# zhuzilin/ring-flash-attention

Hardware: NVIDIA B200
Metric: zigzag_ring_flash_attn_qkvpacked_func fwd_bwd iter/s (higher is better)
Workload: dtype bf16

## Files before the change

### ring_flash_attn_b200/csrc/attn_bwd_sm100.cu

```cuda
#include <math_constants.h>
#include <stdio.h>

#include "attn_common.h"
#include "comm_device.cuh"
#include "sm100_ptx.cuh"

namespace rfa {
namespace bwd {

#ifdef RFA_TRACE
#define RFA_STAMP(cond, iter, slot)                                                              \
  do {                                                                                            \
    if ((cond) && cta == 0 && p.trace != nullptr && (iter) < 64) p.trace[(iter)*16 + (slot)] = clock64(); \
  } while (0)
#else
#define RFA_STAMP(cond, iter, slot) \
  do {                              \
  } while (0)
#endif

constexpr int kTileK = 128;
constexpr int kTileQ = 64;
constexpr int kStages = 3;
constexpr int kThreads = 512;
constexpr int kQHalf = kTileQ * 128;
constexpr int kKVHalf = kTileK * 128;
constexpr int kDSBytes = kTileK * kTileQ * 2;
template <int kD>
struct Geo {
  static constexpr int kKVBytes = kTileK * kD * 2;
  static constexpr int kQBytes = kTileQ * kD * 2;
  static constexpr int kDQBytes = kTileQ * kD * 4;
  static constexpr int kSmemBytes = 2 * kKVBytes + kStages * 2 * kQBytes + kDSBytes + kDQBytes +
                                    kStages * 2 * kTileQ * 4  + 1024  + 1024 ;
};
constexpr uint32_t kTmemCols = 512;
constexpr uint32_t kColS = 0, kColDP = 128, kColDQ = 192, kColDV = 256, kColDK = 384;

struct Barriers {
  uint64_t kv_full;
  uint64_t qdo_full[kStages];
  uint64_t qdo_empty[kStages];
  uint64_t stat_full[kStages];
  uint64_t s_full[2];
  uint64_t p_ready[2];
  uint64_t dp_full;
  uint64_t ds_ready;
  uint64_t dq_full;
  uint64_t dq_free;
  uint64_t dkv_done;
  uint32_t tmem_base;
  uint32_t pad;
};

constexpr int kStatBytes = kStages * 2 * kTileQ * 4;

struct QGeom {
  int q_row0, q_len, diag, lo;
  int t_begin, t_end;
};
__device__ __forceinline__ QGeom q_geom(const BwdQSegment& s) {
  QGeom g;
  g.q_row0 = s.q_row0;
  g.q_len = s.q_len;
  g.diag = s.diag;
  g.lo = s.lo;
  const int first = s.diag >= 0 ? 0 : -s.diag;
  g.t_begin = first / kTileQ;
  g.t_end = (s.q_len + kTileQ - 1) / kTileQ;
  if (g.t_begin > g.t_end) g.t_begin = g.t_end;
  return g;
}

template <typename T, bool kWindow, int kD>
__global__ void __launch_bounds__(kThreads, 1)
attn_bwd_kernel(const __grid_constant__ CUtensorMap tm_q, const __grid_constant__ CUtensorMap tm_do,
                const __grid_constant__ CUtensorMap tm_k, const __grid_constant__ CUtensorMap tm_v,
                const __grid_constant__ CUtensorMap tm_ks, const __grid_constant__ CUtensorMap tm_vs,
                const __grid_constant__ CUtensorMap tm_dq, const __grid_constant__ BwdParams p) {
  if (static_cast<int>(blockIdx.x) < p.push.n_ctas) {
    if (p.push.use_tma) {
      extern __shared__ uint8_t push_smem_raw[];
      push_role_tma(p.push, reinterpret_cast<uint8_t*>((reinterpret_cast<uintptr_t>(push_smem_raw) + 1023) & ~uintptr_t(1023)));
    } else {
      push_role(p.push);
    }
    return;
  }
  static_assert(kD == 64 || kD == 128, "head dim 64 or 128");
  constexpr int kKVBytes = Geo<kD>::kKVBytes, kQBytes = Geo<kD>::kQBytes, kDQBytes = Geo<kD>::kDQBytes;
  constexpr int kSubTiles = kD / 64;
  const int cta = static_cast<int>(blockIdx.x) - p.push.n_ctas;
  extern __shared__ uint8_t smem_raw[];
  uint8_t* smem = reinterpret_cast<uint8_t*>((reinterpret_cast<uintptr_t>(smem_raw) + 1023) & ~uintptr_t(1023));
  uint8_t* smem_k = smem;
  uint8_t* smem_v = smem_k + kKVBytes;
  uint8_t* smem_qdo = smem_v + kKVBytes;
  uint8_t* smem_ds = smem_qdo + kStages * 2 * kQBytes;
  float* smem_dq = reinterpret_cast<float*>(smem_ds + kDSBytes);
  float* smem_stat = reinterpret_cast<float*>(reinterpret_cast<uint8_t*>(smem_dq) + kDQBytes);
  Barriers* bars = reinterpret_cast<Barriers*>(reinterpret_cast<uint8_t*>(smem_stat) + kStatBytes);

  const int warp = threadIdx.x >> 5;
  const int lane = threadIdx.x & 31;
  const int kv_head = p.item_major ? cta % p.hkv : cta / p.n_items;
  const int group = p.hq / p.hkv;
  BwdItem it = p.items[p.item_major ? cta / p.hkv : cta % p.n_items];
  if (p.flags & 4) it.seg_count = 0;

  if (warp == 0 && lane == 0) {
    tma_prefetch_desc(&tm_q);
    tma_prefetch_desc(&tm_do);
    tma_prefetch_desc(&tm_k);
    tma_prefetch_desc(&tm_v);
    tma_prefetch_desc(&tm_dq);
    tma_prefetch_desc(&tm_ks);
    tma_prefetch_desc(&tm_vs);
  }
  if (warp == 1 && lane == 0) {
    mbar_init(&bars->kv_full, 1);
    for (int i = 0; i < kStages; ++i) {
      mbar_init(&bars->qdo_full[i], 1);
      mbar_init(&bars->qdo_empty[i], 1);
      mbar_init(&bars->stat_full[i], 1);
    }
    mbar_init(&bars->s_full[0], 1);
    mbar_init(&bars->s_full[1], 1);
    mbar_init(&bars->p_ready[0], 256);
    mbar_init(&bars->p_ready[1], 256);
    mbar_init(&bars->dp_full, 1);
    mbar_init(&bars->ds_ready, 256);
    mbar_init(&bars->dq_full, 1);
    mbar_init(&bars->dq_free, 128);
    mbar_init(&bars->dkv_done, 1);
    fence_mbar_init();
  }
  if (warp == 2) tmem_alloc<kTmemCols>(&bars->tmem_base);
  tc_fence_before();
  __syncthreads();
  tc_fence_after();
  const uint32_t tmem = bars->tmem_base;

  int tiles_per_head = 0;
  for (int si = 0; si < it.seg_count; ++si) {
    const QGeom g = q_geom(p.qsegs[it.seg_begin + si]);
    tiles_per_head += g.t_end - g.t_begin;
  }
  const int total_tiles = tiles_per_head * group;

  if (warp < 4) {
    reg_dealloc<72>();
    if (warp == 0) {
      if (lane == 0 && total_tiles > 0) {
        const bool staged = it.flag >= 0 && p.ready_flags != nullptr;
        if (staged && !(p.flags & 2)) {
          wait_epoch(p.ready_flags + it.flag, p.ready_epoch, "bwd kv ready", p.sig.my_rank, it.flag);
          fence_proxy_async_all();
        }
        const CUtensorMap* mk = staged ? &tm_ks : &tm_k;
        const CUtensorMap* mv = staged ? &tm_vs : &tm_v;
        mbar_arrive_expect_tx(&bars->kv_full, 2 * kKVBytes);
#pragma unroll
        for (int h = 0; h < kSubTiles; ++h) {
          tma_load_3d(smem_k + h * kKVHalf, mk, &bars->kv_full, 64 * h, kv_head, it.kv_row0);
          tma_load_3d(smem_v + h * kKVHalf, mv, &bars->kv_full, 64 * h, kv_head, it.kv_row0);
        }
        uint32_t slot = 0, phase = 0;
        for (int gq = 0; gq < group; ++gq) {
          const int head = kv_head * group + gq;
          for (int si = 0; si < it.seg_count; ++si) {
            const QGeom g = q_geom(p.qsegs[it.seg_begin + si]);
            for (int ti = g.t_begin; ti < g.t_end; ++ti) {
              const int row = g.q_row0 + ti * kTileQ;
              mbar_wait(&bars->qdo_empty[slot], phase ^ 1);
              uint8_t* dq_ = smem_qdo + slot * 2 * kQBytes;
              uint8_t* ddo = dq_ + kQBytes;
              mbar_arrive_expect_tx(&bars->qdo_full[slot], 2 * kQBytes);
#pragma unroll
              for (int h = 0; h < kSubTiles; ++h) {
                tma_load_3d(dq_ + h * kQHalf, &tm_q, &bars->qdo_full[slot], 64 * h, head, row);
                tma_load_3d(ddo + h * kQHalf, &tm_do, &bars->qdo_full[slot], 64 * h, head, row);
              }
              if (++slot == kStages) {
                slot = 0;
                phase ^= 1;
              }
            }
          }
        }
      }
    } else if (warp == 1) {
      if (total_tiles > 0) {
        const bool leader = elect_one();
        constexpr uint32_t fmt = Pack2<T>::kFmt;
        constexpr uint32_t idesc_st = umma_idesc_f16(fmt, kTileK, kTileQ, 0, 0);
        constexpr uint32_t idesc_dv = umma_idesc_f16(fmt, kTileK, kD, 0, 1);
        constexpr uint32_t idesc_dq = umma_idesc_f16(fmt, 128, kTileQ, 1, 1);
        const uint32_t k_base = smem_u32(smem_k), v_base = smem_u32(smem_v);
        const uint32_t qdo_base = smem_u32(smem_qdo), ds_base = smem_u32(smem_ds);

        constexpr uint32_t hi = umma_desc_hi(1024, kSwizzle128B);
        const uint32_t k_km = umma_desc_lo(k_base, 16);
        const uint32_t v_km = umma_desc_lo(v_base, 16);
        const uint32_t k_mn = umma_desc_lo(k_base, kKVHalf);
        const uint32_t ds_km = umma_desc_lo(ds_base, 16);
        const uint32_t q_km0 = umma_desc_lo(qdo_base, 16);
        const uint32_t q_mn0 = umma_desc_lo(qdo_base, kQHalf);
        constexpr uint32_t stage_step = (2 * kQBytes) >> 4, do_step = kQBytes >> 4;

        auto issue_kq = [&](uint32_t d_col, uint32_t a_lo, uint32_t b_lo) {
#pragma unroll
          for (int k = 0; k < kD / 16; ++k) {
            const uint32_t oa = ((k >> 2) * kKVHalf + (k & 3) * 32) >> 4;
            const uint32_t ob = ((k >> 2) * kQHalf + (k & 3) * 32) >> 4;
            umma_ss2(d_col, a_lo + oa, hi, b_lo + ob, hi, idesc_st, k > 0);
          }
        };

        mbar_wait(&bars->kv_full, 0);
        tc_fence_after();

        uint32_t ph_p[2] = {0, 0};
        uint32_t ph_ds = 0, ph_dqfree = 0;
        int issued_s = 0;
        uint32_t s_slot = 0, s_phase = 0;
        auto issue_s = [&]() {
          mbar_wait(&bars->qdo_full[s_slot], s_phase);
          tc_fence_after();
          if (leader) {
            issue_kq(tmem + kColS + (issued_s & 1) * 64, k_km, q_km0 + s_slot * stage_step);
            umma_commit(&bars->s_full[issued_s & 1]);
          }
          ++issued_s;
          if (++s_slot == kStages) {
            s_slot = 0;
            s_phase ^= 1;
          }
        };
        auto issue_dv = [&](int t, uint32_t t_slot) {
          mbar_wait(&bars->p_ready[t & 1], ph_p[t & 1]);
          ph_p[t & 1] ^= 1;
          tc_fence_after();
          const uint32_t do_mn = q_mn0 + t_slot * stage_step + do_step;
          if (leader)
#pragma unroll
            for (int k = 0; k < kTileQ / 16; ++k)
              umma_ts2(tmem + kColDV, tmem + kColS + (t & 1) * 64 + (k >> 1) * 32 + (k & 1) * 8,
                       do_mn + k * (2048 >> 4), hi, idesc_dv, (t > 0 || k > 0) ? 1u : 0u);
        };
        auto next_slot = [](uint32_t sl) { return sl + 1 == kStages ? 0u : sl + 1; };

        issue_s();
        if (leader) {
          issue_kq(tmem + kColDP, v_km, q_km0 + do_step);
          umma_commit(&bars->dp_full);
        }
        if (total_tiles > 1) issue_s();
        issue_dv(0, 0);
        uint32_t slot = 0;
        for (int i = 0; i < total_tiles; ++i) {
          const uint32_t q_mn = q_mn0 + slot * stage_step;
          const uint32_t slot1 = next_slot(slot);
          RFA_STAMP(leader, i, 0);
          mbar_wait(&bars->ds_ready, ph_ds);
          ph_ds ^= 1;
          tc_fence_after();
          RFA_STAMP(leader, i, 1);
          if (i + 1 < total_tiles && leader) {
            issue_kq(tmem + kColDP, v_km, q_km0 + slot1 * stage_step + do_step);
            umma_commit(&bars->dp_full);
          }
          RFA_STAMP(leader, i, 2);
          if (leader) {
#pragma unroll
            for (int k = 0; k < kTileQ / 16; ++k)
              umma_ss2(tmem + kColDK, ds_km + k * (32 >> 4), hi, q_mn + k * (2048 >> 4), hi, idesc_dv,
                       (i > 0 || k > 0) ? 1u : 0u);
          }
          if (i > 0) {
            mbar_wait(&bars->dq_free, ph_dqfree);
            ph_dqfree ^= 1;
            tc_fence_after();
          }
          RFA_STAMP(leader, i, 3);
          if (leader) {
#pragma unroll
            for (int k = 0; k < kTileK / 16; ++k)
              umma_ss2(tmem + kColDQ, k_mn + k * (2048 >> 4), hi, ds_km + k * (2048 >> 4), hi, idesc_dq, k > 0);
            umma_commit(&bars->dq_full);
            umma_commit(&bars->qdo_empty[slot]);
          }
          RFA_STAMP(leader, i, 4);
          if (i + 1 < total_tiles) issue_dv(i + 1, slot1);
          if (i + 2 < total_tiles) issue_s();
          RFA_STAMP(leader, i, 5);
          slot = slot1;
          __syncwarp();
        }
        if (leader) umma_commit(&bars->dkv_done);
        __syncwarp();
      }
    } else if (warp == 3) {
      uint32_t slot = 0, phase = 0;
      for (int gq = 0; gq < group; ++gq) {
        const int head = kv_head * group + gq;
        for (int si = 0; si < it.seg_count; ++si) {
          const QGeom g = q_geom(p.qsegs[it.seg_begin + si]);
          for (int ti = g.t_begin; ti < g.t_end; ++ti) {
            float l2[2], dl[2];
#pragma unroll
            for (int h = 0; h < 2; ++h) {
              const int qi = ti * kTileQ + lane + 32 * h;
              l2[h] = CUDART_INF_F;
              dl[h] = 0.f;
              if (qi < g.q_len) {
                const int row = g.q_row0 + qi;
                const size_t b = row / p.lse_S, sidx = row % p.lse_S;
                const size_t idx = (b * p.hq + head) * static_cast<size_t>(p.lse_S) + sidx;
                const float x = p.lse[idx];
                l2[h] = x == -CUDART_INF_F ? CUDART_INF_F : x * 1.4426950408889634f;
                dl[h] = p.delta[idx];
              }
            }
            mbar_wait(&bars->qdo_empty[slot], phase ^ 1);
            float* st = smem_stat + slot * 2 * kTileQ;
#pragma unroll
            for (int h = 0; h < 2; ++h) {
              st[lane + 32 * h] = l2[h];
              st[kTileQ + lane + 32 * h] = dl[h];
            }
            __syncwarp();
            if (lane == 0) mbar_arrive(&bars->stat_full[slot]);
            if (++slot == kStages) {
              slot = 0;
              phase ^= 1;
            }
          }
        }
      }
    }
  } else if (warp < 12) {
    reg_alloc<144>();
    const int half = (warp - 4) >> 2;
    const int c0 = half * 32;
    const int wg_tid = (threadIdx.x - 128) & 127;
    const int key = wg_tid;
    const bool key_ok = key < it.kv_rows;
    const uint32_t lane_addr = static_cast<uint32_t>((warp & 3) * 32) << 16;
    uint32_t ph_s[2] = {0, 0};
    uint32_t ph_dp = 0;
    uint32_t st_slot = 0, st_phase = 0;
    int i = 0;
    for (int gq = 0; gq < group; ++gq) {
      for (int si = 0; si < it.seg_count; ++si) {
        const QGeom g = q_geom(p.qsegs[it.seg_begin + si]);
        for (int ti = g.t_begin; ti < g.t_end; ++ti, ++i) {
          const float* st = smem_stat + st_slot * 2 * kTileQ + c0;
          mbar_wait(&bars->stat_full[st_slot], st_phase);
          if (++st_slot == kStages) {
            st_slot = 0;
            st_phase ^= 1;
          }
          float lse2[32];
#pragma unroll
          for (int c = 0; c < 32; c += 4) {
            const float4 v4 = *reinterpret_cast<const float4*>(st + c);
            lse2[c] = v4.x; lse2[c + 1] = v4.y; lse2[c + 2] = v4.z; lse2[c + 3] = v4.w;
          }

          const int buf = i & 1;
          const uint32_t t_s = tmem + kColS + buf * 64 + lane_addr;
          mbar_wait(&bars->s_full[buf], ph_s[buf]);
          ph_s[buf] ^= 1;
          tc_fence_after();
          RFA_STAMP(threadIdx.x == 128, i, 6);
          uint32_t sr[32];
          tmem_ld32(t_s + c0, sr);
          tmem_ld_wait();
          const long long first_q = static_cast<long long>(key) - g.diag - static_cast<long long>(ti) * kTileQ;
          const int q_lo = !key_ok ? kTileQ : (first_q < 0 ? 0 : (first_q > kTileQ ? kTileQ : static_cast<int>(first_q)));
          float pr[32];
          if constexpr (kWindow) {
            const long long last_q = static_cast<long long>(key) - g.lo - static_cast<long long>(ti) * kTileQ;
            const int q_hi = last_q < 0 ? 0 : (last_q >= kTileQ ? kTileQ : static_cast<int>(last_q) + 1);
#pragma unroll
            for (int c = 0; c < 32; ++c) {
              const float e = fast_exp2(fmaf(__uint_as_float(sr[c]), p.scale_log2, -lse2[c]));
              pr[c] = ((c0 + c) >= q_lo && (c0 + c) < q_hi) ? e : 0.f;
            }
          } else {
#pragma unroll
            for (int c = 0; c < 32; ++c) {
              const float e = fast_exp2(fmaf(__uint_as_float(sr[c]), p.scale_log2, -lse2[c]));
              pr[c] = (c0 + c) >= q_lo ? e : 0.f;
            }
          }
          {
            uint32_t pk[16];
#pragma unroll
            for (int c = 0; c < 16; ++c) pk[c] = Pack2<T>::pack(pr[2 * c], pr[2 * c + 1]);
            tmem_st16(t_s + c0, pk);
          }
          tmem_st_wait();
          tc_fence_before();
          mbar_arrive(&bars->p_ready[buf]);
          RFA_STAMP(threadIdx.x == 128, i, 7);

          float dlt[32];
#pragma unroll
          for (int c = 0; c < 32; c += 4) {
            const float4 v4 = *reinterpret_cast<const float4*>(st + kTileQ + c);
            dlt[c] = v4.x; dlt[c + 1] = v4.y; dlt[c + 2] = v4.z; dlt[c + 3] = v4.w;
          }

          mbar_wait(&bars->dp_full, ph_dp);
          ph_dp ^= 1;
          tc_fence_after();
          RFA_STAMP(threadIdx.x == 128, i, 8);
          uint32_t dpr[32];
          tmem_ld32(tmem + kColDP + lane_addr + c0, dpr);
          tmem_ld_wait();
          uint8_t* ds_row = smem_ds + key * 128;
          uint32_t ds_pk[16];
#pragma unroll
          for (int c = 0; c < 32; c += 2) {
            const float d0 = pr[c] * (__uint_as_float(dpr[c]) - dlt[c]) * p.scale;
            const float d1 = pr[c + 1] * (__uint_as_float(dpr[c + 1]) - dlt[c + 1]) * p.scale;
            ds_pk[c >> 1] = Pack2<T>::pack(d0, d1);
          }
          if (i > 0) mbar_wait(&bars->dq_full, (i - 1) & 1);
#pragma unroll
          for (int ch = 0; ch < 4; ++ch)
            *reinterpret_cast<uint4*>(ds_row + (((half * 4 + ch) ^ (key & 7)) << 4)) =
                make_uint4(ds_pk[ch * 4], ds_pk[ch * 4 + 1], ds_pk[ch * 4 + 2], ds_pk[ch * 4 + 3]);
          fence_proxy_async_smem();
          tc_fence_before();
          mbar_arrive(&bars->ds_ready);
          RFA_STAMP(threadIdx.x == 128, i, 9);
        }
      }
    }
    const bool remote = p.dkv.world > 0;
    const int row = (remote ? it.out_row0 : it.kv_row0) + key;
    if (remote && wg_tid == 0) {
      wait_epoch(p.dkv.my_pad + kPadInboxFree + it.owner, p.dkv.wait_epoch, "inbox reuse", p.dkv.my_rank, it.owner);
    }
    if (remote) named_bar_sync(1 + half, 128);
    if (total_tiles > 0) {
      mbar_wait(&bars->dkv_done, 0);
      tc_fence_after();
    }
    auto store_rows = [&](auto tag) {
      using O = decltype(tag);
      constexpr int kRowBytes = kD * static_cast<int>(sizeof(O));
      constexpr int kKVBytes = Geo<kD>::kKVBytes, kQBytes = Geo<kD>::kQBytes;
      constexpr int kPitch = kRowBytes + 16;
      static_assert(2 * kTileK * kPitch <= 2 * kKVBytes + kStages * 2 * kQBytes, "staging must fit in K|V|Q/dO");
      uint8_t* mine = smem_k + half * (kTileK * kPitch) + key * kPitch;
      const uint32_t col = tmem + (half == 0 ? kColDK : kColDV) + lane_addr;
#pragma unroll
      for (int c = 0; c < kD; c += 32) {
        uint32_t r[32];
        if (total_tiles > 0) {
          tmem_ld32(col + c, r);
          tmem_ld_wait();
        } else {
#pragma unroll
          for (int e = 0; e < 32; ++e) r[e] = 0;
        }
        if constexpr (sizeof(O) == 4) {
#pragma unroll
          for (int e = 0; e < 32; e += 4)
            *reinterpret_cast<uint4*>(mine + (c + e) * 4) = make_uint4(r[e], r[e + 1], r[e + 2], r[e + 3]);
        } else {
#pragma unroll
          for (int e = 0; e < 32; e += 8) {
            uint4 v;
            v.x = Pack2<T>::pack(__uint_as_float(r[e + 0]), __uint_as_float(r[e + 1]));
            v.y = Pack2<T>::pack(__uint_as_float(r[e + 2]), __uint_as_float(r[e + 3]));
            v.z = Pack2<T>::pack(__uint_as_float(r[e + 4]), __uint_as_float(r[e + 5]));
            v.w = Pack2<T>::pack(__uint_as_float(r[e + 6]), __uint_as_float(r[e + 7]));
            *reinterpret_cast<uint4*>(mine + (c + e) * 2) = v;
          }
        }
      }
      fence_proxy_async_smem();
      if (key_ok) {
        uint8_t* base = static_cast<uint8_t*>(remote ? (half == 0 ? p.dkv.dk_ptrs[it.owner] : p.dkv.dv_ptrs[it.owner])
                                                     : (half == 0 ? p.dk : p.dv));
        bulk_store(base + (static_cast<size_t>(row) * p.hkv + kv_head) * kRowBytes, mine, kRowBytes);
        tma_store_commit();
        tma_store_wait<0>();
        fence_proxy_async_all();
      }
    };
    if (p.dkv_fp32) store_rows(float{});
    else store_rows(T{});
    if (remote) {
      __threadfence_system();
      named_bar_sync(3, 256);
      if (half == 0 && wg_tid == 0) {
        const uint32_t old = atomicAdd(p.dkv.sent_count + it.owner, 1u);
        if (old + 1u == p.dkv.sent_target[it.owner]) {
          __threadfence_system();
          st_release_sys(p.dkv.peer_pads[it.owner] + kPadDkvReady + p.dkv.my_rank, p.dkv.epoch);
        }
      }
    }
  } else {
    reg_alloc<144>();
    const int wg_tid = threadIdx.x - 384;
    const uint32_t lane_addr = static_cast<uint32_t>((warp & 3) * 32) << 16;
    uint32_t ph = 0;
    int i = 0;
    for (int gq = 0; gq < group; ++gq) {
      const int head = kv_head * group + gq;
      for (int si = 0; si < it.seg_count; ++si) {
        const QGeom g = q_geom(p.qsegs[it.seg_begin + si]);
        for (int ti = g.t_begin; ti < g.t_end; ++ti, ++i) {
          mbar_wait(&bars->dq_full, ph);
          ph ^= 1;
          tc_fence_after();
          RFA_STAMP(wg_tid == 0, i, 11);
          uint32_t r[64];
          tmem_ld32(tmem + kColDQ + lane_addr, r);
          tmem_ld32(tmem + kColDQ + lane_addr + 32, r + 32);
          tmem_ld_wait();
          tc_fence_before();
          mbar_arrive(&bars->dq_free);
          if (wg_tid == 0) tma_store_wait_read<0>();
          named_bar_sync(4, 128);
          if (wg_tid < kD) {
#pragma unroll
            for (int q = 0; q < kTileQ; ++q) smem_dq[q * kD + wg_tid] = __uint_as_float(r[q]);
          }
          fence_proxy_async_smem();
          named_bar_sync(4, 128);
          if (wg_tid == 0) {
            tma_reduce_add_3d(&tm_dq, smem_dq, 0, head, g.q_row0 + ti * kTileQ);
            tma_store_commit();
          }
          RFA_STAMP(wg_tid == 0, i, 12);
        }
      }
    }
    if (wg_tid == 0) tma_store_wait<0>();
  }

  tc_fence_before();
  __syncthreads();
  if (warp == 2) tmem_dealloc<kTmemCols>(tmem);
  if (threadIdx.x == 0 && p.sig.world > 0) consumer_done(p.sig);
}

template <typename T>
__global__ void bwd_delta_kernel(const T* __restrict__ out, const T* __restrict__ dout, float* __restrict__ delta,
                                 int rows, int hq, int lse_S, int64_t o_rs, int64_t o_hs, int64_t do_rs,
                                 int64_t do_hs, int head_dim) {
  const int gw = (blockIdx.x * blockDim.x + threadIdx.x) >> 5;
  const int lane = threadIdx.x & 31;
  if (gw >= rows * hq) return;
  const int row = gw / hq, head = gw % hq;
  float s = 0.f;
  if (lane * 4 < head_dim) {
    const uint2 a = *reinterpret_cast<const uint2*>(out + row * o_rs + head * o_hs + lane * 4);
    const uint2 b = *reinterpret_cast<const uint2*>(dout + row * do_rs + head * do_hs + lane * 4);
    const T* pa = reinterpret_cast<const T*>(&a);
    const T* pb = reinterpret_cast<const T*>(&b);
#pragma unroll
    for (int i = 0; i < 4; ++i) s += static_cast<float>(pa[i]) * static_cast<float>(pb[i]);
  }
#pragma unroll
  for (int o = 16; o > 0; o >>= 1) s += __shfl_xor_sync(0xffffffffu, s, o);
  if (lane == 0) {
    const size_t b_ = row / lse_S, sidx = row % lse_S;
    delta[(b_ * hq + head) * static_cast<size_t>(lse_S) + sidx] = s;
  }
}

}

const char* attn_bwd_delta_launch(int dtype, const TensorView& out, const TensorView& dout, float* delta, int lse_S,
                                  int head_dim, cudaStream_t stream) {
  const int rows = static_cast<int>(out.rows), hq = out.heads;
  const long long warps = static_cast<long long>(rows) * hq;
  if (warps == 0) return nullptr;
  const int threads = 256;
  const int blocks = static_cast<int>((warps * 32 + threads - 1) / threads);
  if (dtype == kDtypeBF16) {
    bwd::bwd_delta_kernel<__nv_bfloat16><<<blocks, threads, 0, stream>>>(
        static_cast<const __nv_bfloat16*>(out.ptr), static_cast<const __nv_bfloat16*>(dout.ptr), delta, rows, hq, lse_S,
        out.row_stride, out.head_stride, dout.row_stride, dout.head_stride, head_dim);
  } else {
    bwd::bwd_delta_kernel<__half><<<blocks, threads, 0, stream>>>(
        static_cast<const __half*>(out.ptr), static_cast<const __half*>(dout.ptr), delta, rows, hq, lse_S,
        out.row_stride, out.head_stride, dout.row_stride, dout.head_stride, head_dim);
  }
  cudaError_t err = cudaGetLastError();
  return err == cudaSuccess ? nullptr : cudaGetErrorString(err);
}

const char* attn_bwd_launch(int dtype, const TensorView& q, const TensorView& dout, const TensorView& k,
                            const TensorView& v, const TensorView& k_stage, const TensorView& v_stage,
                            const TensorView& dq_accum, const BwdParams& p, cudaStream_t stream) {
  const int n_blocks = p.push.n_ctas + p.n_items * p.hkv;
  if (n_blocks <= 0) return nullptr;
  if (p.sig.world > 0) set_peer_timeout_from_env();
  CUtensorMap tq, tdo, tk, tv, tks, tvs, tdq;
  const int d = p.head_dim;
  if (d != 64 && d != 128) return "the sm_100a backward is instantiated for head_dim 64 and 128";
  if (const char* e = make_tensor_map(&tq, q, 2, bwd::kTileQ, d)) return e;
  if (const char* e = make_tensor_map(&tdo, dout, 2, bwd::kTileQ, d)) return e;
  if (const char* e = make_tensor_map(&tk, k, 2, bwd::kTileK, d)) return e;
  if (const char* e = make_tensor_map(&tv, v, 2, bwd::kTileK, d)) return e;
  if (const char* e = make_tensor_map(&tks, k_stage, 2, bwd::kTileK, d)) return e;
  if (const char* e = make_tensor_map(&tvs, v_stage, 2, bwd::kTileK, d)) return e;
  if (const char* e = make_plain_tensor_map(&tdq, dq_accum, 4, bwd::kTileQ, d)) return e;
  dim3 grid(n_blocks, 1, 1), block(bwd::kThreads, 1, 1);
  cudaError_t err;
  err = cudaSuccess;
  auto launch = [&](auto kern, int smem) {
    if (p.push.n_ctas > 0 && smem < kPushSmemBytes) smem = kPushSmemBytes;
    err = cudaFuncSetAttribute(kern, cudaFuncAttributeMaxDynamicSharedMemorySize, smem);
    if (err == cudaSuccess) kern<<<grid, block, smem, stream>>>(tq, tdo, tk, tv, tks, tvs, tdq, p);
  };
  auto pick = [&](auto tag) {
    using T = decltype(tag);
    if (d == 128) {
      if (p.window) launch(bwd::attn_bwd_kernel<T, true, 128>, bwd::Geo<128>::kSmemBytes);
      else launch(bwd::attn_bwd_kernel<T, false, 128>, bwd::Geo<128>::kSmemBytes);
    } else {
      if (p.window) launch(bwd::attn_bwd_kernel<T, true, 64>, bwd::Geo<64>::kSmemBytes);
      else launch(bwd::attn_bwd_kernel<T, false, 64>, bwd::Geo<64>::kSmemBytes);
    }
  };
  if (dtype == kDtypeBF16) pick(__nv_bfloat16{});
  else pick(__half{});
  if (err != cudaSuccess) return cudaGetErrorString(err);
  err = cudaGetLastError();
  return err == cudaSuccess ? nullptr : cudaGetErrorString(err);
}

}
```

Before: 27.80.

## Double-buffer dS and reuse S TMEM for dQ, stage V in TMEM

The kernel now double-buffers the dS^T shared-memory tile, placing the second buffer in the V tile's space. To make that space free, V is copied once into TMEM so dP is computed with a TMEM-operand MMA. The dQ accumulator now reuses the current S slot in TMEM, with per-buffer dq_full, ds_free and dv_done barriers. The aim is to let softmax warps write the next dS while the dQ/dK MMAs still read the previous one, removing a serialization point. The cost is added barrier traffic and a tighter ordering between the dV MMA finishing and dQ overwriting S, which is a correctness risk.

```diff
diff --git a/ring_flash_attn_b200/csrc/attn_bwd_sm100.cu b/ring_flash_attn_b200/csrc/attn_bwd_sm100.cu
--- a/ring_flash_attn_b200/csrc/attn_bwd_sm100.cu
+++ b/ring_flash_attn_b200/csrc/attn_bwd_sm100.cu
@@ -35,7 +35,7 @@
                                     kStages * 2 * kTileQ * 4  + 1024  + 1024 ;
 };
 constexpr uint32_t kTmemCols = 512;
-constexpr uint32_t kColS = 0, kColDP = 128, kColDQ = 192, kColDV = 256, kColDK = 384;
+constexpr uint32_t kColS = 0, kColDP = 128, kColV = 192, kColDV = 256, kColDK = 384;
 
 struct Barriers {
   uint64_t kv_full;
@@ -44,9 +44,12 @@
   uint64_t stat_full[kStages];
   uint64_t s_full[2];
   uint64_t p_ready[2];
+  uint64_t v_ready;
   uint64_t dp_full;
   uint64_t ds_ready;
-  uint64_t dq_full;
+  uint64_t dq_full[2];
+  uint64_t ds_free[2];
+  uint64_t dv_done[2];
   uint64_t dq_free;
   uint64_t dkv_done;
   uint32_t tmem_base;
@@ -96,8 +99,10 @@
   uint8_t* smem_k = smem;
   uint8_t* smem_v = smem_k + kKVBytes;
   uint8_t* smem_qdo = smem_v + kKVBytes;
-  uint8_t* smem_ds = smem_qdo + kStages * 2 * kQBytes;
-  float* smem_dq = reinterpret_cast<float*>(smem_ds + kDSBytes);
+  uint8_t* smem_ds0 = smem_qdo + kStages * 2 * kQBytes;
+  uint8_t* smem_ds1 = smem_v;
+  static_assert(kKVBytes >= kDSBytes, "dS^T buffer 1 must fit in the V tile");
+  float* smem_dq = reinterpret_cast<float*>(smem_ds0 + kDSBytes);
   float* smem_stat = reinterpret_cast<float*>(reinterpret_cast<uint8_t*>(smem_dq) + kDQBytes);
   Barriers* bars = reinterpret_cast<Barriers*>(reinterpret_cast<uint8_t*>(smem_stat) + kStatBytes);
 
@@ -128,9 +133,15 @@
     mbar_init(&bars->s_full[1], 1);
     mbar_init(&bars->p_ready[0], 256);
     mbar_init(&bars->p_ready[1], 256);
+    mbar_init(&bars->v_ready, 256);
     mbar_init(&bars->dp_full, 1);
     mbar_init(&bars->ds_ready, 256);
-    mbar_init(&bars->dq_full, 1);
+    mbar_init(&bars->dq_full[0], 1);
+    mbar_init(&bars->dq_full[1], 1);
+    mbar_init(&bars->ds_free[0], 1);
+    mbar_init(&bars->ds_free[1], 1);
+    mbar_init(&bars->dv_done[0], 1);
+    mbar_init(&bars->dv_done[1], 1);
     mbar_init(&bars->dq_free, 128);
     mbar_init(&bars->dkv_done, 1);
     fence_mbar_init();
@@ -196,31 +207,38 @@
         constexpr uint32_t idesc_st = umma_idesc_f16(fmt, kTileK, kTileQ, 0, 0);
         constexpr uint32_t idesc_dv = umma_idesc_f16(fmt, kTileK, kD, 0, 1);
         constexpr uint32_t idesc_dq = umma_idesc_f16(fmt, 128, kTileQ, 1, 1);
-        const uint32_t k_base = smem_u32(smem_k), v_base = smem_u32(smem_v);
-        const uint32_t qdo_base = smem_u32(smem_qdo), ds_base = smem_u32(smem_ds);
+        const uint32_t k_base = smem_u32(smem_k), qdo_base = smem_u32(smem_qdo);
 
         constexpr uint32_t hi = umma_desc_hi(1024, kSwizzle128B);
         const uint32_t k_km = umma_desc_lo(k_base, 16);
-        const uint32_t v_km = umma_desc_lo(v_base, 16);
         const uint32_t k_mn = umma_desc_lo(k_base, kKVHalf);
-        const uint32_t ds_km = umma_desc_lo(ds_base, 16);
+        const uint32_t ds_km[2] = {umma_desc_lo(smem_u32(smem_ds0), 16),
+                                   umma_desc_lo(smem_u32(smem_ds1), 16)};
         const uint32_t q_km0 = umma_desc_lo(qdo_base, 16);
         const uint32_t q_mn0 = umma_desc_lo(qdo_base, kQHalf);
         constexpr uint32_t stage_step = (2 * kQBytes) >> 4, do_step = kQBytes >> 4;
 
-        auto issue_kq = [&](uint32_t d_col, uint32_t a_lo, uint32_t b_lo) {
+        auto issue_s_mma = [&](uint32_t d_col, uint32_t b_lo) {
 #pragma unroll
           for (int k = 0; k < kD / 16; ++k) {
             const uint32_t oa = ((k >> 2) * kKVHalf + (k & 3) * 32) >> 4;
             const uint32_t ob = ((k >> 2) * kQHalf + (k & 3) * 32) >> 4;
-            umma_ss2(d_col, a_lo + oa, hi, b_lo + ob, hi, idesc_st, k > 0);
-          }
+            umma_ss2(d_col, k_km + oa, hi, b_lo + ob, hi, idesc_st, k > 0);
+          }
+        };
+        auto issue_dp = [&](uint32_t b_lo) {
+#pragma unroll
+          for (int k = 0; k < kD / 16; ++k) {
+            const uint32_t ob = ((k >> 2) * kQHalf + (k & 3) * 32) >> 4;
+            umma_ts2(tmem + kColDP, tmem + kColV + k * 8, b_lo + ob, hi, idesc_st, k > 0);
+          }
+          umma_commit(&bars->dp_full);
         };
 
         mbar_wait(&bars->kv_full, 0);
         tc_fence_after();
 
-        uint32_t ph_p[2] = {0, 0};
+        uint32_t ph_p[2] = {0, 0}, ph_dv[2] = {0, 0};
         uint32_t ph_ds = 0, ph_dqfree = 0;
         int issued_s = 0;
         uint32_t s_slot = 0, s_phase = 0;
@@ -228,7 +246,7 @@
           mbar_wait(&bars->qdo_full[s_slot], s_phase);
           tc_fence_after();
           if (leader) {
-            issue_kq(tmem + kColS + (issued_s & 1) * 64, k_km, q_km0 + s_slot * stage_step);
+            issue_s_mma(tmem + kColS + (issued_s & 1) * 64, q_km0 + s_slot * stage_step);
             umma_commit(&bars->s_full[issued_s & 1]);
           }
           ++issued_s;
@@ -242,57 +260,63 @@
           ph_p[t & 1] ^= 1;
           tc_fence_after();
           const uint32_t do_mn = q_mn0 + t_slot * stage_step + do_step;
-          if (leader)
+          if (leader) {
 #pragma unroll
             for (int k = 0; k < kTileQ / 16; ++k)
               umma_ts2(tmem + kColDV, tmem + kColS + (t & 1) * 64 + (k >> 1) * 32 + (k & 1) * 8,
                        do_mn + k * (2048 >> 4), hi, idesc_dv, (t > 0 || k > 0) ? 1u : 0u);
+            umma_commit(&bars->dv_done[t & 1]);
+          }
         };
         auto next_slot = [](uint32_t sl) { return sl + 1 == kStages ? 0u : sl + 1; };
 
         issue_s();
-        if (leader) {
-          issue_kq(tmem + kColDP, v_km, q_km0 + do_step);
-          umma_commit(&bars->dp_full);
-        }
+        mbar_wait(&bars->v_ready, 0);
+        tc_fence_after();
+        if (leader) issue_dp(q_km0 + do_step);
         if (total_tiles > 1) issue_s();
         issue_dv(0, 0);
         uint32_t slot = 0;
         for (int i = 0; i < total_tiles; ++i) {
           const uint32_t q_mn = q_mn0 + slot * stage_step;
           const uint32_t slot1 = next_slot(slot);
+          const uint32_t ds_i = ds_km[i & 1];
           RFA_STAMP(leader, i, 0);
           mbar_wait(&bars->ds_ready, ph_ds);
           ph_ds ^= 1;
           tc_fence_after();
           RFA_STAMP(leader, i, 1);
-          if (i + 1 < total_tiles && leader) {
-            issue_kq(tmem + kColDP, v_km, q_km0 + slot1 * stage_step + do_step);
-            umma_commit(&bars->dp_full);
-          }
+          if (i + 1 < total_tiles && leader)
+            issue_dp(q_km0 + slot1 * stage_step + do_step);
           RFA_STAMP(leader, i, 2);
+          mbar_wait(&bars->dv_done[i & 1], ph_dv[i & 1]);
+          ph_dv[i & 1] ^= 1;
+          tc_fence_after();
           if (leader) {
 #pragma unroll
+            for (int k = 0; k < kTileK / 16; ++k)
+              umma_ss2(tmem + kColS + (i & 1) * 64, k_mn + k * (2048 >> 4), hi, ds_i + k * (2048 >> 4), hi,
+                       idesc_dq, k > 0);
+            umma_commit(&bars->dq_full[i & 1]);
+          }
+          RFA_STAMP(leader, i, 3);
+          if (leader) {
+#pragma unroll
             for (int k = 0; k < kTileQ / 16; ++k)
-              umma_ss2(tmem + kColDK, ds_km + k * (32 >> 4), hi, q_mn + k * (2048 >> 4), hi, idesc_dv,
+              umma_ss2(tmem + kColDK, ds_i + k * (32 >> 4), hi, q_mn + k * (2048 >> 4), hi, idesc_dv,
                        (i > 0 || k > 0) ? 1u : 0u);
-          }
-          if (i > 0) {
+            umma_commit(&bars->ds_free[i & 1]);
+            umma_commit(&bars->qdo_empty[slot]);
+          }
+          RFA_STAMP(leader, i, 4);
+          if (i + 1 < total_tiles) issue_dv(i + 1, slot1);
+          if (i + 2 < total_tiles) {
             mbar_wait(&bars->dq_free, ph_dqfree);
             ph_dqfree ^= 1;
             tc_fence_after();
-          }
-          RFA_STAMP(leader, i, 3);
-          if (leader) {
-#pragma unroll
-            for (int k = 0; k < kTileK / 16; ++k)
-              umma_ss2(tmem + kColDQ, k_mn + k * (2048 >> 4), hi, ds_km + k * (2048 >> 4), hi, idesc_dq, k > 0);
-            umma_commit(&bars->dq_full);
-            umma_commit(&bars->qdo_empty[slot]);
-          }
-          RFA_STAMP(leader, i, 4);
-          if (i + 1 < total_tiles) issue_dv(i + 1, slot1);
-          if (i + 2 < total_tiles) issue_s();
+            RFA_STAMP(leader, i, 13);
+            issue_s();
+          }
           RFA_STAMP(leader, i, 5);
           slot = slot1;
           __syncwarp();
@@ -347,6 +371,24 @@
     const int key = wg_tid;
     const bool key_ok = key < it.kv_rows;
     const uint32_t lane_addr = static_cast<uint32_t>((warp & 3) * 32) << 16;
+    if (total_tiles > 0) {
+      mbar_wait(&bars->kv_full, 0);
+#pragma unroll
+      for (int h = 0; h < kSubTiles; ++h) {
+        uint32_t vr[16];
+        const uint8_t* vrow = smem_v + h * kKVHalf + key * 128;
+#pragma unroll
+        for (int ch = 0; ch < 4; ++ch) {
+          const uint4 v4 = *reinterpret_cast<const uint4*>(vrow + (((half * 4 + ch) ^ (key & 7)) << 4));
+          vr[ch * 4] = v4.x; vr[ch * 4 + 1] = v4.y; vr[ch * 4 + 2] = v4.z; vr[ch * 4 + 3] = v4.w;
+        }
+        tmem_st16(tmem + kColV + lane_addr + h * 32 + half * 16, vr);
+      }
+      tmem_st_wait();
+      tc_fence_before();
+      mbar_arrive(&bars->v_ready);
+      mbar_wait(&bars->v_ready, 0);
+    }
     uint32_t ph_s[2] = {0, 0};
     uint32_t ph_dp = 0;
     uint32_t st_slot = 0, st_phase = 0;
@@ -420,7 +462,7 @@
           uint32_t dpr[32];
           tmem_ld32(tmem + kColDP + lane_addr + c0, dpr);
           tmem_ld_wait();
-          uint8_t* ds_row = smem_ds + key * 128;
+          uint8_t* ds_row = ((i & 1) ? smem_ds1 : smem_ds0) + key * 128;
           uint32_t ds_pk[16];
 #pragma unroll
           for (int c = 0; c < 32; c += 2) {
@@ -428,7 +470,7 @@
             const float d1 = pr[c + 1] * (__uint_as_float(dpr[c + 1]) - dlt[c + 1]) * p.scale;
             ds_pk[c >> 1] = Pack2<T>::pack(d0, d1);
           }
-          if (i > 0) mbar_wait(&bars->dq_full, (i - 1) & 1);
+          if (i > 1) mbar_wait(&bars->ds_free[i & 1], ((i >> 1) - 1) & 1);
 #pragma unroll
           for (int ch = 0; ch < 4; ++ch)
             *reinterpret_cast<uint4*>(ds_row + (((half * 4 + ch) ^ (key & 7)) << 4)) =
@@ -511,20 +553,19 @@
     reg_alloc<144>();
     const int wg_tid = threadIdx.x - 384;
     const uint32_t lane_addr = static_cast<uint32_t>((warp & 3) * 32) << 16;
-    uint32_t ph = 0;
     int i = 0;
     for (int gq = 0; gq < group; ++gq) {
       const int head = kv_head * group + gq;
       for (int si = 0; si < it.seg_count; ++si) {
         const QGeom g = q_geom(p.qsegs[it.seg_begin + si]);
         for (int ti = g.t_begin; ti < g.t_end; ++ti, ++i) {
-          mbar_wait(&bars->dq_full, ph);
-          ph ^= 1;
+          mbar_wait(&bars->dq_full[i & 1], (i >> 1) & 1);
           tc_fence_after();
           RFA_STAMP(wg_tid == 0, i, 11);
           uint32_t r[64];
-          tmem_ld32(tmem + kColDQ + lane_addr, r);
-          tmem_ld32(tmem + kColDQ + lane_addr + 32, r + 32);
+          const uint32_t t_dq = tmem + kColS + (i & 1) * 64 + lane_addr;
+          tmem_ld32(t_dq, r);
+          tmem_ld32(t_dq + 32, r + 32);
           tmem_ld_wait();
           tc_fence_before();
           mbar_arrive(&bars->dq_free);
```

Result: no change. 27.95, median of 6 (+0.5%).
